# NetManAIOps/ChatTS

Measured on NVIDIA H100. Metric: decode_tokens_per_s, higher is better.
Workload: dtype bf16

## Files before the change

chatts_b200/csrc/common.cuh:

```cuda
#pragma once
#include <cuda.h>
#include <cudaTypedefs.h>
#include <cuda_bf16.h>
#include <cuda_fp16.h>
#include <cuda_runtime.h>
#include <stdint.h>
#include <stdio.h>
#include <string.h>

#include "../../include/chatts_b200.h"

struct cts_ctx {
  int device;
  int sm_count;
  int max_smem_optin;
  char err[512];
  void* scratch;
  size_t scratch_bytes;
  PFN_cuTensorMapEncodeTiled_v12000 encode_tiled;
  int l2_prefetch_mb;
  int no_persistent_gemm;
  int norm_cluster;
  int decode_stages;
  int no_ts_fused;
  int no_next_prefetch;
  int next_prefetch_mb;
};

int cts_set_error(cts_ctx* ctx, int code, const char* fmt, ...);

#define CTS_CHECK_ARG(ctx, cond, msg)                                         \
  do {                                                                        \
    if (!(cond)) return cts_set_error((ctx), CTS_ERR_BAD_ARG, "%s: %s", __func__, (msg)); \
  } while (0)

#define CTS_CUDA(ctx, expr)                                                   \
  do {                                                                        \
    cudaError_t _e = (expr);                                                  \
    if (_e != cudaSuccess)                                                    \
      return cts_set_error((ctx), CTS_ERR_CUDA, "%s: %s -> %s", __func__, #expr, cudaGetErrorString(_e)); \
  } while (0)

#define CTS_LAUNCH_CHECK(ctx)                                                 \
  do {                                                                        \
    cudaError_t _e = cudaGetLastError();                                      \
    if (_e != cudaSuccess)                                                    \
      return cts_set_error((ctx), CTS_ERR_CUDA, "%s: launch -> %s", __func__, cudaGetErrorString(_e)); \
  } while (0)

static inline long long cdiv_ll(long long a, long long b) { return (a + b - 1) / b; }

__device__ __forceinline__ void pdl_wait() { asm volatile("griddepcontrol.wait;" ::: "memory"); }
__device__ __forceinline__ void pdl_trigger() { asm volatile("griddepcontrol.launch_dependents;" ::: "memory"); }

template <typename... KArgs, typename... Args>
static inline cudaError_t launch_pdl(void (*kern)(KArgs...), dim3 grid, dim3 block, size_t smem, cudaStream_t st,
                                     unsigned cluster_x, Args... args) {
  cudaLaunchConfig_t cfg = {};
  cfg.gridDim = grid;
  cfg.blockDim = block;
  cfg.dynamicSmemBytes = smem;
  cfg.stream = st;
  cudaLaunchAttribute attr[2];
  int n = 0;
  attr[n].id = cudaLaunchAttributeProgrammaticStreamSerialization;
  attr[n].val.programmaticStreamSerializationAllowed = 1;
  ++n;
  if (cluster_x > 1) {
    attr[n].id = cudaLaunchAttributeClusterDimension;
    attr[n].val.clusterDim.x = cluster_x;
    attr[n].val.clusterDim.y = 1;
    attr[n].val.clusterDim.z = 1;
    ++n;
  }
  cfg.attrs = attr;
  cfg.numAttrs = n;
  return cudaLaunchKernelEx(&cfg, kern, static_cast<KArgs>(args)...);
}

template <typename T> struct DT;
template <> struct DT<__nv_bfloat16> {
  static __device__ __forceinline__ float to_f(__nv_bfloat16 v) { return __bfloat162float(v); }
  static __device__ __forceinline__ __nv_bfloat16 from_f(float v) { return __float2bfloat16_rn(v); }
};
template <> struct DT<__half> {
  static __device__ __forceinline__ float to_f(__half v) { return __half2float(v); }
  static __device__ __forceinline__ __half from_f(float v) { return __float2half_rn(v); }
};
template <typename T> __device__ __forceinline__ float rnd(float v) { return DT<T>::to_f(DT<T>::from_f(v)); }

template <typename T> __device__ __forceinline__ void unpack8(const uint4& u, float* f) {
  const T* p = reinterpret_cast<const T*>(&u);
#pragma unroll
  for (int i = 0; i < 8; ++i) f[i] = DT<T>::to_f(p[i]);
}
template <typename T> __device__ __forceinline__ uint4 pack8(const float* f) {
  uint4 u;
  T* p = reinterpret_cast<T*>(&u);
#pragma unroll
  for (int i = 0; i < 8; ++i) p[i] = DT<T>::from_f(f[i]);
  return u;
}

__device__ __forceinline__ float warp_sum(float v) {
#pragma unroll
  for (int o = 16; o > 0; o >>= 1) v += __shfl_xor_sync(0xffffffffu, v, o);
  return v;
}
__device__ __forceinline__ float warp_max(float v) {
#pragma unroll
  for (int o = 16; o > 0; o >>= 1) v = fmaxf(v, __shfl_xor_sync(0xffffffffu, v, o));
  return v;
}

__device__ __forceinline__ float gelu_erf(float x) { return 0.5f * x * (1.0f + erff(x * 0.70710678118654752440f)); }
__device__ __forceinline__ float silu_f(float x) { return x / (1.0f + expf(-x)); }

__device__ __forceinline__ uint32_t smem_u32(const void* p) { return (uint32_t)__cvta_generic_to_shared(p); }

__device__ __forceinline__ void mbar_init(uint64_t* bar, uint32_t count) {
  asm volatile("mbarrier.init.shared::cta.b64 [%0], %1;" ::"r"(smem_u32(bar)), "r"(count) : "memory");
}
__device__ __forceinline__ void fence_mbar_init() { asm volatile("fence.mbarrier_init.release.cluster;" ::: "memory"); }
__device__ __forceinline__ void fence_proxy_async_smem() { asm volatile("fence.proxy.async.shared::cta;" ::: "memory"); }

__device__ __forceinline__ void mbar_expect_tx(uint64_t* bar, uint32_t bytes) {
  asm volatile("mbarrier.arrive.expect_tx.shared::cta.b64 _, [%0], %1;" ::"r"(smem_u32(bar)), "r"(bytes) : "memory");
}
__device__ __forceinline__ void mbar_arrive(uint64_t* bar) {
  asm volatile("mbarrier.arrive.shared::cta.b64 _, [%0];" ::"r"(smem_u32(bar)) : "memory");
}
__device__ __forceinline__ bool mbar_try_wait(uint64_t* bar, uint32_t parity) {
  uint32_t ok;
  asm volatile(
      "{\n\t.reg .pred p;\n\t"
      "mbarrier.try_wait.parity.shared::cta.b64 p, [%1], %2;\n\t"
      "selp.u32 %0, 1, 0, p;\n\t}"
      : "=r"(ok)
      : "r"(smem_u32(bar)), "r"(parity)
      : "memory");
  return ok != 0;
}
#ifndef CTS_WAIT_LIMIT
#define CTS_WAIT_LIMIT (1u << 26)
#endif
__device__ __forceinline__ void mbar_wait(uint64_t* bar, uint32_t parity) {
  uint32_t n = 0;
  while (!mbar_try_wait(bar, parity)) {
    if (++n > CTS_WAIT_LIMIT) {
      printf("chatts_b200: mbarrier wait timed out (block %d,%d,%d thread %d)\n", blockIdx.x, blockIdx.y, blockIdx.z,
             threadIdx.x);
      __trap();
    }
  }
}

#define CTS_L2_EVICT_NORMAL 0x1000000000000000ull
#define CTS_L2_EVICT_FIRST 0x12F0000000000000ull
#define CTS_L2_EVICT_LAST 0x14F0000000000000ull

__device__ __forceinline__ void tma_load_2d(void* smem_dst, const CUtensorMap* tm, uint64_t* bar, int c0, int c1,
                                            uint64_t policy) {
  asm volatile(
      "cp.async.bulk.tensor.2d.shared::cluster.global.mbarrier::complete_tx::bytes.L2::cache_hint"
      " [%0], [%1, {%3, %4}], [%2], %5;"
      ::"r"(smem_u32(smem_dst)), "l"(tm), "r"(smem_u32(bar)), "r"(c0), "r"(c1), "l"(policy)
      : "memory");
}
__device__ __forceinline__ void tma_prefetch_l2_2d(const CUtensorMap* tm, int c0, int c1) {
  asm volatile("cp.async.bulk.prefetch.tensor.2d.L2.global.tile [%0, {%1, %2}];" ::"l"(tm), "r"(c0), "r"(c1) : "memory");
}
__device__ __forceinline__ void tma_store_2d(const CUtensorMap* tm, const void* smem_src, int c0, int c1) {
  asm volatile("cp.async.bulk.tensor.2d.global.shared::cta.bulk_group [%0, {%2, %3}], [%1];"
               ::"l"(tm), "r"(smem_u32(smem_src)), "r"(c0), "r"(c1) : "memory");
}
__device__ __forceinline__ void tma_store_commit() { asm volatile("cp.async.bulk.commit_group;" ::: "memory"); }
__device__ __forceinline__ void tma_store_wait_read0() { asm volatile("cp.async.bulk.wait_group 0;" ::: "memory"); }
__device__ __forceinline__ void tma_load_2d_nohint(void* smem_dst, const CUtensorMap* tm, uint64_t* bar, int c0, int c1) {
  asm volatile(
// ... 168 lines not shown
```

chatts_b200/csrc/ctx.cu:

```cuda
#include <stdarg.h>
#include <stdlib.h>

#include "common.cuh"
#include "tensormap.cuh"

int cts_set_error(cts_ctx* ctx, int code, const char* fmt, ...) {
  if (ctx) {
    va_list ap;
    va_start(ap, fmt);
    vsnprintf(ctx->err, sizeof(ctx->err), fmt, ap);
    va_end(ap);
  }
  return code;
}

extern "C" int cts_version(void) { return 100; }

extern "C" const char* cts_arch(void) {
#if defined(CTS_BUILD_ARCH)
  return CTS_BUILD_ARCH;
#else
  return "unknown";
#endif
}

extern "C" int cts_ctx_create(int device, cts_ctx** out) {
  if (!out) return CTS_ERR_BAD_ARG;
  *out = nullptr;
  cts_ctx* ctx = (cts_ctx*)calloc(1, sizeof(cts_ctx));
  if (!ctx) return CTS_ERR_CUDA;
  ctx->device = device;
  cudaError_t e = cudaSetDevice(device);
  if (e != cudaSuccess) {
    fprintf(stderr, "chatts_b200: cudaSetDevice(%d) failed: %s\n", device, cudaGetErrorString(e));
    free(ctx);
    return CTS_ERR_CUDA;
  }
  cudaDeviceProp prop;
  e = cudaGetDeviceProperties(&prop, device);
  if (e != cudaSuccess) {
    free(ctx);
    return CTS_ERR_CUDA;
  }
  if (prop.major != 9 || prop.minor != 0) {
    fprintf(stderr, "chatts_b200: device %d is sm_%d%d; this library contains sm_90a code only\n", device, prop.major,
            prop.minor);
    free(ctx);
    return CTS_ERR_UNSUPPORTED;
  }
  ctx->sm_count = prop.multiProcessorCount;
  ctx->max_smem_optin = (int)prop.sharedMemPerBlockOptin;
  void* fn = nullptr;
  cudaDriverEntryPointQueryResult qres;
  e = cudaGetDriverEntryPoint("cuTensorMapEncodeTiled", &fn, cudaEnableDefault, &qres);
  if (e != cudaSuccess || qres != cudaDriverEntryPointSuccess || !fn) {
    fprintf(stderr, "chatts_b200: cannot resolve cuTensorMapEncodeTiled\n");
    free(ctx);
    return CTS_ERR_CUDA;
  }
  ctx->encode_tiled = (PFN_cuTensorMapEncodeTiled_v12000)fn;
  const char* e1 = getenv("CTS_L2_PREFETCH_MB");
  ctx->l2_prefetch_mb = e1 ? atoi(e1) : 0;
  const char* e4 = getenv("CTS_NO_PERSISTENT_GEMM");
  ctx->no_persistent_gemm = e4 ? atoi(e4) : 0;
  const char* e5 = getenv("CTS_NORM_CLUSTER");
  ctx->norm_cluster = e5 ? atoi(e5) : 8;
  const char* e2 = getenv("CTS_DECODE_SMEM_KB");
  ctx->decode_stages = e2 ? atoi(e2) : 75;
  {
    int cur = 0;
    cudaGetDevice(&cur);
    cudaSetDevice(device);
    ctx->scratch = nullptr;
    ctx->scratch_bytes = 4096;
    if (cudaMalloc(&ctx->scratch, ctx->scratch_bytes) != cudaSuccess || cudaMemset(ctx->scratch, 0, ctx->scratch_bytes) != cudaSuccess) {
      fprintf(stderr, "chatts_b200: cannot allocate the context scratch\n");
      ctx->scratch = nullptr;
    }
    cudaSetDevice(cur);
  }
  const char* e8 = getenv("CTS_TS_FUSED");
  ctx->no_ts_fused = (e8 && atoi(e8) == 0) ? 1 : 0;
  const char* e6 = getenv("CTS_NEXT_PREFETCH");
  ctx->no_next_prefetch = (e6 && atoi(e6) == 0) ? 1 : 0;
  const char* e7 = getenv("CTS_NEXT_PREFETCH_MB");
  ctx->next_prefetch_mb = e7 ? atoi(e7) : 0;
  *out = ctx;
  return CTS_OK;
}

extern "C" void cts_ctx_destroy(cts_ctx* ctx) {
  if (!ctx) return;
  if (ctx->scratch) cudaFree(ctx->scratch);
  free(ctx);
}

extern "C" const char* cts_last_error(const cts_ctx* ctx) { return ctx ? ctx->err : "null ctx"; }

int cts_make_tmap_2d(cts_ctx* ctx, CUtensorMap* tm, const void* base, long long rows, long long cols, long long ld_elems,
                     int box_rows, int is_bf16) {
  if (((uintptr_t)base & 15) != 0) return cts_set_error(ctx, CTS_ERR_BAD_ARG, "tensor map: base not 16-byte aligned");
  if ((ld_elems * 2) % 16 != 0) return cts_set_error(ctx, CTS_ERR_BAD_ARG, "tensor map: row pitch %lld B not a multiple of 16", ld_elems * 2);
  if (box_rows < 1 || box_rows > 256) return cts_set_error(ctx, CTS_ERR_BAD_ARG, "tensor map: box rows %d", box_rows);
  cuuint64_t dims[2] = {(cuuint64_t)cols, (cuuint64_t)rows};
  cuuint64_t strides[1] = {(cuuint64_t)(ld_elems * 2)};
  cuuint32_t box[2] = {64u, (cuuint32_t)box_rows};
  cuuint32_t estr[2] = {1u, 1u};
  CUresult r = ctx->encode_tiled(tm, is_bf16 ? CU_TENSOR_MAP_DATA_TYPE_BFLOAT16 : CU_TENSOR_MAP_DATA_TYPE_FLOAT16, 2,
                                 const_cast<void*>(base), dims, strides, box, estr, CU_TENSOR_MAP_INTERLEAVE_NONE,
                                 CU_TENSOR_MAP_SWIZZLE_128B, CU_TENSOR_MAP_L2_PROMOTION_L2_256B,
                                 CU_TENSOR_MAP_FLOAT_OOB_FILL_NONE);
  if (r != CUDA_SUCCESS) return cts_set_error(ctx, CTS_ERR_CUDA, "cuTensorMapEncodeTiled failed: CUresult %d", (int)r);
  return CTS_OK;
}

int cts_make_tmap_2d_dense(cts_ctx* ctx, CUtensorMap* tm, const void* base, long long rows, long long cols, long long ld_elems,
                           int box_rows, int box_cols, int is_bf16) {
  if (((uintptr_t)base & 15) != 0) return cts_set_error(ctx, CTS_ERR_BAD_ARG, "tensor map: base not 16-byte aligned");
  if ((ld_elems * 2) % 16 != 0) return cts_set_error(ctx, CTS_ERR_BAD_ARG, "tensor map: row pitch %lld B not a multiple of 16", ld_elems * 2);
  if (box_rows < 1 || box_rows > 256 || box_cols < 8 || box_cols > 256 || (box_cols * 2) % 16 != 0)
    return cts_set_error(ctx, CTS_ERR_BAD_ARG, "tensor map: box %d x %d", box_rows, box_cols);
  cuuint64_t dims[2] = {(cuuint64_t)cols, (cuuint64_t)rows};
  cuuint64_t strides[1] = {(cuuint64_t)(ld_elems * 2)};
  cuuint32_t box[2] = {(cuuint32_t)box_cols, (cuuint32_t)box_rows};
  cuuint32_t estr[2] = {1u, 1u};
  CUresult r = ctx->encode_tiled(tm, is_bf16 ? CU_TENSOR_MAP_DATA_TYPE_BFLOAT16 : CU_TENSOR_MAP_DATA_TYPE_FLOAT16, 2,
                                 const_cast<void*>(base), dims, strides, box, estr, CU_TENSOR_MAP_INTERLEAVE_NONE,
                                 CU_TENSOR_MAP_SWIZZLE_NONE, CU_TENSOR_MAP_L2_PROMOTION_L2_256B, CU_TENSOR_MAP_FLOAT_OOB_FILL_NONE);
  if (r != CUDA_SUCCESS) return cts_set_error(ctx, CTS_ERR_CUDA, "cuTensorMapEncodeTiled (dense) failed: CUresult %d", (int)r);
  return CTS_OK;
}

extern "C" int cts_trace_set_gemm(unsigned long long* buf);
extern "C" int cts_trace_set_elementwise(unsigned long long* buf);
extern "C" int cts_trace_set_attention(unsigned long long* buf);
extern "C" int cts_trace_set_allreduce_ll(unsigned long long* buf);
extern "C" int cts_trace_set_fused(unsigned long long* buf);
extern "C" int cts_trace_set_ts_fused(unsigned long long* buf);
extern "C" int cts_trace_set_w4(unsigned long long* buf);
extern "C" int cts_trace_enable(cts_ctx* ctx, unsigned long long* buf) {
  if (!ctx) return CTS_ERR_BAD_ARG;
  if (cts_trace_set_gemm(buf) || cts_trace_set_elementwise(buf) || cts_trace_set_attention(buf) || cts_trace_set_allreduce_ll(buf) || cts_trace_set_fused(buf) || cts_trace_set_ts_fused(buf) || cts_trace_set_w4(buf))
    return cts_set_error(ctx, CTS_ERR_CUDA, "cts_trace_enable: cudaMemcpyToSymbol failed");
  return CTS_OK;
}
```

chatts_b200/csrc/gemm_tcgen05.cu:

```cuda
#include <type_traits>

#include "common.cuh"
#include "tensormap.cuh"
#include "trace.cuh"

namespace {

constexpr int kBM = 128;
constexpr int kBK = 64;
constexpr int kMaxStages = 12;
constexpr int kThreads = 192;

struct GemmParams {
  long long n, k, t, out_ld;
  const void* bias;
  const void* residual;
  void* out;
  const int* row_map;
  int kb_total;
  int split_k;
  int stages;
  int epilogue;
  float* splitk_ws;
  int* tile_cnt;
  int l2_prefetch;
  int staged;
  int next_tiles, next_split, next_kb_total, next_pf;
};

template <int BN, bool DUAL> __host__ __device__ constexpr int stage_bytes() { return kBM * kBK * 2 * (DUAL ? 2 : 1) + BN * kBK * 2; }
template <int BN> __host__ __device__ constexpr bool acc_in_ring() { return BN <= 32; }

template <typename T, int BN, bool DUAL>
__global__ void __launch_bounds__(kThreads, 1)
gemm_tn_kernel(const __grid_constant__ CUtensorMap tm_w, const __grid_constant__ CUtensorMap tm_w2,
               const __grid_constant__ CUtensorMap tm_x, const __grid_constant__ CUtensorMap tm_next, const __grid_constant__ CUtensorMap tm_out,
               const __grid_constant__ CUtensorMap tm_res, const GemmParams p) {
  extern __shared__ uint8_t smem_raw[];
  __shared__ uint64_t full_bar[kMaxStages];
  __shared__ uint64_t empty_bar[kMaxStages];
  __shared__ uint64_t res_bar;
  __shared__ int last_flag;

  constexpr int kStage = stage_bytes<BN, DUAL>();
  constexpr int kABytes = kBM * kBK * 2;
  constexpr int kLd = acc_ld<BN>();
  constexpr bool kIsBf16 = std::is_same<T, __nv_bfloat16>::value;

  const uint32_t raw = smem_u32(smem_raw);
  uint8_t* smem = smem_raw + (((raw + 1023u) & ~1023u) - raw);

  const int warp = threadIdx.x >> 5;
  const int lane = threadIdx.x & 31;
  const int f0 = blockIdx.x * kBM;
  const int t0 = blockIdx.y * BN;
  const int split = blockIdx.z;
  const int stages = p.stages;

  const int kb0 = (int)(((long long)p.kb_total * split) / p.split_k);
  const int kb1 = (int)(((long long)p.kb_total * (split + 1)) / p.split_k);
  const int nkb = kb1 - kb0;

  pdl_trigger();
  if (threadIdx.x == 0) {
    tma_prefetch_desc(&tm_w);
    tma_prefetch_desc(&tm_x);
    if (DUAL) tma_prefetch_desc(&tm_w2);
    for (int s = 0; s < stages; ++s) {
      mbar_init(&full_bar[s], 1);
      mbar_init(&empty_bar[s], 1);
    }
    mbar_init(&res_bar, 1);
    fence_mbar_init();
  }
  __syncthreads();

  if (warp == 4) {
    if (lane == 0) {
      const int npre = nkb < stages ? nkb : stages;
      CTS_TRACE(CTS_TK_GEMM, 0);
      for (int i = 0; i < npre; ++i) {
        mbar_expect_tx(&full_bar[i], (uint32_t)kStage);
        uint8_t* st = smem + (size_t)i * kStage;
        const int kc = (kb0 + i) * kBK;
        tma_load_2d(st, &tm_w, &full_bar[i], kc, f0, CTS_L2_EVICT_FIRST);
        if (DUAL) tma_load_2d(st + kABytes, &tm_w2, &full_bar[i], kc, f0, CTS_L2_EVICT_FIRST);
      }
      {
        const int npf = (nkb - npre) < p.l2_prefetch ? (nkb - npre) : p.l2_prefetch;
        for (int i = npre; i < npre + npf; ++i) {
          tma_prefetch_l2_2d(&tm_w, (kb0 + i) * kBK, f0);
          if (DUAL) tma_prefetch_l2_2d(&tm_w2, (kb0 + i) * kBK, f0);
        }
      }
      pdl_wait();
      CTS_TRACE(CTS_TK_GEMM, 1);
      for (int i = 0; i < npre; ++i) {
        uint8_t* st = smem + (size_t)i * kStage;
        tma_load_2d(st + kABytes * (DUAL ? 2 : 1), &tm_x, &full_bar[i], (kb0 + i) * kBK, t0, CTS_L2_EVICT_LAST);
      }
      for (int i = npre; i < nkb; ++i) {
        const int s = i % stages;
        const uint32_t ph = (uint32_t)(i / stages) & 1u;
        mbar_wait(&empty_bar[s], ph ^ 1u);
        mbar_expect_tx(&full_bar[s], (uint32_t)kStage);
        uint8_t* st = smem + (size_t)s * kStage;
        const int kc = (kb0 + i) * kBK;
        tma_load_2d(st, &tm_w, &full_bar[s], kc, f0, CTS_L2_EVICT_FIRST);
        if (DUAL) tma_load_2d(st + kABytes, &tm_w2, &full_bar[s], kc, f0, CTS_L2_EVICT_FIRST);
        tma_load_2d(st + kABytes * (DUAL ? 2 : 1), &tm_x, &full_bar[s], kc, t0, CTS_L2_EVICT_LAST);
      }
      CTS_TRACE(CTS_TK_GEMM, 2);
      if (p.next_pf > 0) {
        const int units = p.next_tiles * p.next_split;
        const int n_ours = (int)(gridDim.x * gridDim.y * gridDim.z);
        const int c = (int)(blockIdx.x + gridDim.x * (blockIdx.y + gridDim.y * blockIdx.z));
        for (int u = c; u < units; u += n_ours) {
          const int x2 = u % p.next_tiles, z2 = u / p.next_tiles;
          const int kbn0 = (int)(((long long)p.next_kb_total * z2) / p.next_split);
          const int kbn1 = (int)(((long long)p.next_kb_total * (z2 + 1)) / p.next_split);
          const int cnt = (kbn1 - kbn0) < p.next_pf ? (kbn1 - kbn0) : p.next_pf;
          for (int i = 0; i < cnt; ++i) tma_prefetch_l2_2d(&tm_next, (kbn0 + i) * kBK, x2 * kBM);
        }
      }
    }
  } else if (warp < 4) {
    Acc128<BN> acc, acc2;
    acc.zero();
    if (DUAL) acc2.zero();
    for (int i = 0; i < nkb; ++i) {
      const int s = i % stages;
      mbar_wait(&full_bar[s], (uint32_t)(i / stages) & 1u);
      const uint32_t a_addr = smem_u32(smem + (size_t)s * kStage);
      const uint32_t b_addr = a_addr + kABytes * (DUAL ? 2 : 1);
      acc.template mma_kblock<kIsBf16>(a_addr, b_addr, i == 0);
      if (DUAL) acc2.template mma_kblock<kIsBf16>(a_addr + kABytes, b_addr, i == 0);
      wgmma_wait<DUAL ? 2 : 1>();
      if (i > 0 && threadIdx.x == 0) mbar_arrive(&empty_bar[(i - 1) % stages]);
    }
    wgmma_wait<0>();
    if (nkb > 0 && threadIdx.x == 0) mbar_arrive(&empty_bar[(nkb - 1) % stages]);
    named_bar_sync(1, 128);
    float* acc_s = reinterpret_cast<float*>(acc_in_ring<BN>() ? smem : smem + (size_t)stages * kStage);
    acc.store(acc_s, kLd);
    if (DUAL) acc2.store(acc_s + kBM * kLd, kLd);
    pdl_wait();
    named_bar_sync(1, 128);
    const int q = warp & 3;
    const long long f = (long long)f0 + q * 32 + lane;
    const bool f_ok = f < p.n;
    const int row = q * 32 + lane;
    float bias = 0.f;
    if (p.bias != nullptr && f_ok) bias = DT<T>::to_f(reinterpret_cast<const T*>(p.bias)[f]);
    const int epi = p.epilogue;
    if (p.staged) {
      T* out_s = reinterpret_cast<T*>(smem);
      T* res_s = reinterpret_cast<T*>(smem + (size_t)BN * kBM * 2);
      const int ft = q * 32 + lane;
      if (epi == CTS_EPI_RESIDUAL) {
        if (threadIdx.x == 64) {
          mbar_expect_tx(&res_bar, (uint32_t)(BN * kBM * 2));
          tma_load_2d_nohint(res_s, &tm_res, &res_bar, f0, t0);
        }
        mbar_wait(&res_bar, 0);
      }
#pragma unroll 1
      for (int c = 0; c < BN; c += 16) {
        if ((long long)t0 + c >= p.t) break;
        uint32_t v[16], v2[16];
        acc_ld16(acc_s, kLd, row, c, v);
        if (DUAL) acc_ld16(acc_s + kBM * kLd, kLd, row, c, v2);
#pragma unroll
        for (int j = 0; j < 16; ++j) {
          const float acc = __uint_as_float(v[j]);
          float r;
          if (epi == CTS_EPI_SWIGLU) {
            r = rnd<T>(silu_f(rnd<T>(acc))) * rnd<T>(__uint_as_float(v2[j]));
          } else {
            r = acc + bias;
            if (epi == CTS_EPI_GELU) r = gelu_erf(rnd<T>(r));
            else if (epi == CTS_EPI_RESIDUAL) r = rnd<T>(r) + DT<T>::to_f(res_s[(c + j) * kBM + ft]);
          }
          out_s[(c + j) * kBM + ft] = DT<T>::from_f(r);
        }
      }
      fence_proxy_async_smem();
      named_bar_sync(1, 128);
      if (threadIdx.x == 64) {
        tma_store_2d(&tm_out, out_s, f0, t0);
        tma_store_commit();
        tma_store_wait_read0();
      }
    } else if (epi == CTS_EPI_SPLITK_F32) {
      float* dst = p.split_k > 1 ? p.splitk_ws + (long long)split * p.t * p.n : reinterpret_cast<float*>(p.out);
#pragma unroll 1
      for (int c = 0; c < BN; c += 16) {
        if ((long long)t0 + c >= p.t) break;
        uint32_t v[16];
        acc_ld16(acc_s, kLd, row, c, v);
#pragma unroll
        for (int j = 0; j < 16; ++j) {
          const long long t = (long long)t0 + c + j;
          if (t < p.t && f_ok) dst[t * p.n + f] = __uint_as_float(v[j]);
        }
      }
      if (p.split_k > 1) {
        __threadfence();
        named_bar_sync(1, 128);
        const int tile_id = blockIdx.y * gridDim.x + blockIdx.x;
        if (threadIdx.x == 64) last_flag = (atomicAdd(&p.tile_cnt[tile_id], 1) == p.split_k - 1);
        named_bar_sync(1, 128);
        if (last_flag) {
          __threadfence();
          const long long tmax = p.t - t0 < BN ? p.t - t0 : BN;
          if (f_ok) {
            float* o = reinterpret_cast<float*>(p.out);
#pragma unroll 2
            for (long long tt = 0; tt < tmax; ++tt) {
              const long long off = (t0 + tt) * p.n + f;
              float a = 0.f;
              for (int s2 = 0; s2 < p.split_k; ++s2) a += __ldcg(p.splitk_ws + (long long)s2 * p.t * p.n + off);
              o[off] = a;
            }
          }
          if (threadIdx.x == 64) p.tile_cnt[tile_id] = 0;
        }
      }
    } else {
#pragma unroll 1
    for (int c = 0; c < BN; c += 16) {
      if ((long long)t0 + c >= p.t) break;
      uint32_t v[16], v2[16];
      acc_ld16(acc_s, kLd, row, c, v);
      if (DUAL) acc_ld16(acc_s + kBM * kLd, kLd, row, c, v2);
#pragma unroll
      for (int j = 0; j < 16; ++j) {
        const long long t = (long long)t0 + c + j;
        if (t >= p.t || !f_ok) continue;
        const float acc = __uint_as_float(v[j]);
        if (epi == CTS_EPI_PARTIAL_F32) {
          reinterpret_cast<float*>(p.out)[((long long)split * p.t + t) * p.n + f] = acc;
          continue;
        }
        long long row = t;
        if (p.row_map != nullptr) {
          row = p.row_map[t];
          if (row < 0) continue;
        }
        float r;
        if (epi == CTS_EPI_SWIGLU) {
          const float g = rnd<T>(acc);
          const float u = rnd<T>(__uint_as_float(v2[j]));
          r = rnd<T>(silu_f(g)) * u;
        } else {
          r = acc + bias;
          if (epi == CTS_EPI_GELU) {
            r = gelu_erf(rnd<T>(r));
          } else if (epi == CTS_EPI_RESIDUAL) {
            r = rnd<T>(r) + DT<T>::to_f(reinterpret_cast<const T*>(p.residual)[row * p.out_ld + f]);
          }
        }
        reinterpret_cast<T*>(p.out)[row * p.out_ld + f] = DT<T>::from_f(r);
      }
    }
    }
  }

  if (threadIdx.x == 0) CTS_TRACE(CTS_TK_GEMM, 3);
}

constexpr int kPBN = 128;
constexpr int kPStages = 4;
constexpr int kPStageBytes = kBM * kBK * 2 + kPBN * kBK * 2;
constexpr int kPOutBytes = kPBN * kBM * 2;

template <typename T>
__global__ void __launch_bounds__(kThreads, 1)
gemm_tn_persistent_kernel(const __grid_constant__ CUtensorMap tm_w, const __grid_constant__ CUtensorMap tm_x,
                          const __grid_constant__ CUtensorMap tm_out, const __grid_constant__ CUtensorMap tm_res,
                          const GemmParams p) {
  extern __shared__ uint8_t smem_raw[];
  __shared__ uint64_t full_bar[kPStages], empty_bar[kPStages], res_bar;
  constexpr bool kIsBf16 = std::is_same<T, __nv_bfloat16>::value;
  const uint32_t raw = smem_u32(smem_raw);
  uint8_t* smem = smem_raw + (((raw + 1023u) & ~1023u) - raw);
  uint8_t* out_s = smem + kPStages * kPStageBytes;
  uint8_t* res_s = out_s + kPOutBytes;

  const int warp = threadIdx.x >> 5, lane = threadIdx.x & 31;
  const int tiles_m = (int)((p.n + kBM - 1) / kBM), tiles_n = (int)((p.t + kPBN - 1) / kPBN);
  const int total_tiles = tiles_m * tiles_n;
  const int nkb = p.kb_total;
  const int epi = p.epilogue;
  const int gm = p.l2_prefetch > 0 ? p.l2_prefetch : tiles_m;
  auto tile_coords = [&](int id, int& m_blk, int& n_blk) {
    const int per_group = gm * tiles_n;
    const int g = id / per_group, r = id - g * per_group;
    const int gm_here = min(gm, tiles_m - g * gm);
    n_blk = r / gm_here;
    m_blk = g * gm + (r - n_blk * gm_here);
  };

  pdl_trigger();
  if (threadIdx.x == 0) {
    tma_prefetch_desc(&tm_w); tma_prefetch_desc(&tm_x); tma_prefetch_desc(&tm_out);
    for (int s = 0; s < kPStages; ++s) { mbar_init(&full_bar[s], 1); mbar_init(&empty_bar[s], 1); }
    mbar_init(&res_bar, 1);
    fence_mbar_init();
  }
  __syncthreads();

  if (warp == 4) {
    if (lane == 0) {
      pdl_wait();
      uint32_t it = 0;
      for (int tile = blockIdx.x; tile < total_tiles; tile += gridDim.x) {
        int mb, nb;
        tile_coords(tile, mb, nb);
        const int f0 = mb * kBM, t0 = nb * kPBN;
        for (int kb = 0; kb < nkb; ++kb, ++it) {
          const int s = it % kPStages;
          mbar_wait(&empty_bar[s], ((it / kPStages) & 1u) ^ 1u);
          mbar_expect_tx(&full_bar[s], (uint32_t)kPStageBytes);
          uint8_t* st = smem + (size_t)s * kPStageBytes;
          tma_load_2d(st, &tm_w, &full_bar[s], kb * kBK, f0, CTS_L2_EVICT_NORMAL);
          tma_load_2d(st + kBM * kBK * 2, &tm_x, &full_bar[s], kb * kBK, t0, CTS_L2_EVICT_NORMAL);
        }
      }
    }
  } else if (warp < 4) {
    pdl_wait();
    uint32_t it = 0, res_uses = 0;
    T* outp = reinterpret_cast<T*>(out_s);
    const T* resp = reinterpret_cast<const T*>(res_s);
    const T* biasp = reinterpret_cast<const T*>(p.bias);
    for (int tile = blockIdx.x; tile < total_tiles; tile += gridDim.x) {
      int mb, nb;
      tile_coords(tile, mb, nb);
      const int f0 = mb * kBM, t0 = nb * kPBN;
      if (epi == CTS_EPI_RESIDUAL && threadIdx.x == 0) {
        fence_proxy_async_smem();
        mbar_expect_tx(&res_bar, (uint32_t)kPOutBytes);
        tma_load_2d_nohint(res_s, &tm_res, &res_bar, f0, t0);
      }
      Acc128<kPBN> acc;
      acc.zero();
      for (int kb = 0; kb < nkb; ++kb, ++it) {
        const int s = it % kPStages;
        mbar_wait(&full_bar[s], (it / kPStages) & 1u);
        const uint32_t a_addr = smem_u32(smem + (size_t)s * kPStageBytes);
        acc.template mma_kblock<kIsBf16>(a_addr, a_addr + kBM * kBK * 2, kb == 0);
        wgmma_wait<1>();
        if (kb > 0 && threadIdx.x == 0) mbar_arrive(&empty_bar[(it - 1) % kPStages]);
      }
      wgmma_wait<0>();
      if (nkb > 0 && threadIdx.x == 0) mbar_arrive(&empty_bar[(it - 1) % kPStages]);
      if (epi == CTS_EPI_RESIDUAL) {
        mbar_wait(&res_bar, res_uses & 1u);
        ++res_uses;
      }
      if (epi == CTS_EPI_SWIGLU_IL) {
#pragma unroll
        for (int i = 0; i < kPBN / 2; ++i) {
          const float g = rnd<T>(acc.d[0][i]);
          const float u = rnd<T>(acc.d[1][i]);
          outp[acc_col(i) * 64 + acc_row(i)] = DT<T>::from_f(rnd<T>(silu_f(g)) * u);
        }
      } else {
#pragma unroll
        for (int h = 0; h < 2; ++h) {
          float bias[2] = {0.f, 0.f};
#pragma unroll
          for (int e = 0; e < 2; ++e) {
            const long long f = (long long)f0 + 64 * h + acc_row(2 * e);
            if (biasp != nullptr && f < p.n) bias[e] = DT<T>::to_f(biasp[f]);
          }
#pragma unroll
          for (int i = 0; i < kPBN / 2; ++i) {
            const int ft = 64 * h + acc_row(i), tt = acc_col(i);
            float r = acc.d[h][i] + bias[(i >> 1) & 1];
            if (epi == CTS_EPI_GELU) r = gelu_erf(rnd<T>(r));
            else if (epi == CTS_EPI_RESIDUAL) r = rnd<T>(r) + DT<T>::to_f(resp[tt * kBM + ft]);
            outp[tt * kBM + ft] = DT<T>::from_f(r);
          }
        }
      }
      fence_proxy_async_smem();
      named_bar_sync(1, 128);
      if (threadIdx.x == 0) {
        if (epi == CTS_EPI_SWIGLU_IL) tma_store_2d(&tm_out, out_s, f0 / 2, t0);
        else tma_store_2d(&tm_out, out_s, f0, t0);
        tma_store_commit();
        asm volatile("cp.async.bulk.wait_group.read 0;" ::: "memory");
      }
      named_bar_sync(1, 128);
    }
    if (threadIdx.x == 0) tma_store_wait_read0();
  }
}

template <typename T>
int launch_persistent(cts_ctx* ctx, const cts_gemm_args* a, cudaStream_t stream) {
  const bool is_bf16 = a->dtype == CTS_BF16;
  const bool il = a->epilogue == CTS_EPI_SWIGLU_IL;
  CUtensorMap tm_w, tm_x, tm_out, tm_res;
  int rc = cts_make_tmap_2d(ctx, &tm_w, a->w, a->n, a->k, a->w_ld, kBM, is_bf16);
  if (rc) return rc;
  rc = cts_make_tmap_2d(ctx, &tm_x, a->x, a->t, a->k, a->x_ld, kPBN, is_bf16);
  if (rc) return rc;
  rc = cts_make_tmap_2d_dense(ctx, &tm_out, a->out, a->t, il ? a->n / 2 : a->n, a->out_ld, kPBN, il ? 64 : kBM, is_bf16);
  if (rc) return rc;
  tm_res = tm_out;
  if (a->epilogue == CTS_EPI_RESIDUAL) {
    rc = cts_make_tmap_2d_dense(ctx, &tm_res, a->residual, a->t, a->n, a->out_ld, kPBN, kBM, is_bf16);
    if (rc) return rc;
  }
  GemmParams p;
  memset(&p, 0, sizeof(p));
  p.n = a->n; p.k = a->k; p.t = a->t; p.out_ld = a->out_ld;
  p.bias = a->bias; p.residual = a->residual; p.out = a->out;
  p.kb_total = (int)cdiv_ll(a->k, kBK);
  p.split_k = 1; p.epilogue = a->epilogue; p.stages = kPStages;
  {
    const long long tiles_m = cdiv_ll(a->n, kBM);
    long long gmax = (20LL << 20) / ((long long)kBM * a->k * 2);
    if (gmax < 1) gmax = 1;
    const long long groups = cdiv_ll(tiles_m, gmax);
    p.l2_prefetch = (int)cdiv_ll(tiles_m, groups);
    if (ctx->l2_prefetch_mb < 0) p.l2_prefetch = 0;
  }
  const size_t smem = (size_t)kPStages * kPStageBytes + 2 * kPOutBytes + 1024;
  auto kern = gemm_tn_persistent_kernel<T>;
  CTS_CUDA(ctx, cudaFuncSetAttribute(kern, cudaFuncAttributeMaxDynamicSharedMemorySize, (int)smem));
  const long long tiles = cdiv_ll(a->n, kBM) * cdiv_ll(a->t, kPBN);
  const unsigned grid = (unsigned)(tiles < ctx->sm_count ? tiles : ctx->sm_count);
  CTS_CUDA(ctx, launch_pdl(kern, dim3(grid), dim3(kThreads), smem, stream, 1, tm_w, tm_x, tm_out, tm_res, p));
  return CTS_OK;
}

template <typename T, int BN, bool DUAL>
int launch(cts_ctx* ctx, const cts_gemm_args* a, cudaStream_t stream) {
  const bool is_bf16 = a->dtype == CTS_BF16;
  CUtensorMap tm_w, tm_w2, tm_x;
  int rc = cts_make_tmap_2d(ctx, &tm_w, a->w, a->n, a->k, a->w_ld, kBM, is_bf16);
  if (rc) return rc;
  if (DUAL) {
    rc = cts_make_tmap_2d(ctx, &tm_w2, a->w2, a->n, a->k, a->w_ld, kBM, is_bf16);
    if (rc) return rc;
  } else {
    tm_w2 = tm_w;
  }
  rc = cts_make_tmap_2d(ctx, &tm_x, a->x, a->t, a->k, a->x_ld, BN, is_bf16);
  if (rc) return rc;
  const bool staged = BN >= 64 && a->row_map == nullptr && a->epilogue != CTS_EPI_PARTIAL_F32 && a->epilogue != CTS_EPI_SPLITK_F32 && (a->out_ld * 2) % 16 == 0 &&
                      ((uintptr_t)a->out & 15) == 0 && (a->epilogue != CTS_EPI_RESIDUAL || ((uintptr_t)a->residual & 15) == 0);
  CUtensorMap tm_out = tm_x, tm_res = tm_x;
  if (staged) {
    rc = cts_make_tmap_2d_dense(ctx, &tm_out, a->out, a->t, a->n, a->out_ld, BN, kBM, is_bf16);
    if (rc) return rc;
    if (a->epilogue == CTS_EPI_RESIDUAL) {
      rc = cts_make_tmap_2d_dense(ctx, &tm_res, a->residual, a->t, a->n, a->out_ld, BN, kBM, is_bf16);
      if (rc) return rc;
    }
  }

  GemmParams p;
  p.n = a->n; p.k = a->k; p.t = a->t; p.out_ld = a->out_ld;
  p.bias = a->bias; p.residual = a->residual; p.out = a->out; p.row_map = a->row_map;
  p.splitk_ws = (float*)a->splitk_ws; p.tile_cnt = a->tile_counters;
  p.kb_total = (int)cdiv_ll(a->k, kBK);
  p.split_k = a->split_k;
  p.epilogue = a->epilogue;
  CUtensorMap tm_next = tm_w;
  p.next_tiles = p.next_split = p.next_kb_total = p.next_pf = 0;
  if (BN <= 32 && a->next_w != nullptr && a->next_prefetch_bytes > 0 && a->next_n > 0 && a->next_k > 0 && a->next_split >= 1 && !ctx->no_next_prefetch) {
    rc = cts_make_tmap_2d(ctx, &tm_next, a->next_w, a->next_n, a->next_k, a->next_ld > 0 ? a->next_ld : a->next_k, kBM, is_bf16);
    if (rc) return rc;
    p.next_tiles = (int)cdiv_ll(a->next_n, kBM);
    p.next_split = a->next_split;
    p.next_kb_total = (int)cdiv_ll(a->next_k, kBK);
    const long long units = (long long)p.next_tiles * p.next_split;
    long long pf = a->next_prefetch_bytes / (units * kBM * kBK * 2);
    const long long per_unit = cdiv_ll(p.next_kb_total, p.next_split);
    if (pf > per_unit) pf = per_unit;
    p.next_pf = (int)pf;
  }
  constexpr int kStage = stage_bytes<BN, DUAL>();
  const int budget = (BN <= 32) ? ctx->decode_stages * 1024 : (BN <= 128 ? 100 * 1024 : 200 * 1024);
  int stages = budget / kStage;
  if (stages > kMaxStages) stages = kMaxStages;
  if (stages < 2) stages = 2;
  p.stages = stages;
  p.staged = staged ? 1 : 0;
  p.l2_prefetch = 0;
  if (BN <= 32 && ctx->l2_prefetch_mb > 0) {
    const long long ctas = cdiv_ll(a->n, kBM) * cdiv_ll(a->t, BN) * a->split_k;
    const long long per = ((long long)ctx->l2_prefetch_mb << 20) / (ctas * kBM * kBK * 2 * (DUAL ? 2 : 1));
    p.l2_prefetch = (int)(per > 64 ? 64 : per);
  }
  if (staged && stages * kStage < 2 * BN * kBM * 2) stages = (2 * BN * kBM * 2 + kStage - 1) / kStage;
  p.stages = stages;
  const size_t acc_bytes = (size_t)acc_smem_bytes<BN>() * (DUAL ? 2 : 1);
  const size_t ring = (size_t)stages * kStage;
  const size_t smem = (acc_in_ring<BN>() ? (ring > acc_bytes ? ring : acc_bytes) : ring + acc_bytes) + 1024;
  auto kern = gemm_tn_kernel<T, BN, DUAL>;
  CTS_CUDA(ctx, cudaFuncSetAttribute(kern, cudaFuncAttributeMaxDynamicSharedMemorySize, (int)smem));
  dim3 grid((unsigned)cdiv_ll(a->n, kBM), (unsigned)cdiv_ll(a->t, BN), (unsigned)a->split_k);
  CTS_CUDA(ctx, launch_pdl(kern, grid, dim3(kThreads), smem, stream, 1, tm_w, tm_w2, tm_x, tm_next, tm_out, tm_res, p));
  return CTS_OK;
}

template <typename T, bool DUAL>
int dispatch_bn(cts_ctx* ctx, const cts_gemm_args* a, cudaStream_t stream) {
  const long long t = a->t;
  if (t <= 16) return launch<T, 16, DUAL>(ctx, a, stream);
  if (t <= 32) return launch<T, 32, DUAL>(ctx, a, stream);
  if (t <= 64 || DUAL) return launch<T, 64, DUAL>(ctx, a, stream);
  return launch<T, 128, false>(ctx, a, stream);
}

}

extern "C" int cts_gemm(cts_ctx* ctx, const cts_gemm_args* a, void* stream) {
  if (!ctx) return CTS_ERR_BAD_ARG;
  CTS_CHECK_ARG(ctx, a != nullptr, "null args");
  CTS_CHECK_ARG(ctx, a->w && a->x && a->out, "null w/x/out");
  CTS_CHECK_ARG(ctx, a->n > 0 && a->k > 0 && a->t > 0, "n, k, t must be positive");
  CTS_CHECK_ARG(ctx, a->dtype == CTS_BF16 || a->dtype == CTS_F16, "dtype must be CTS_BF16 or CTS_F16");
  CTS_CHECK_ARG(ctx, a->epilogue >= CTS_EPI_NONE && a->epilogue <= CTS_EPI_SWIGLU_IL, "unknown epilogue");
  CTS_CHECK_ARG(ctx, a->split_k >= 1, "split_k must be >= 1");
  CTS_CHECK_ARG(ctx, a->split_k == 1 || a->epilogue == CTS_EPI_PARTIAL_F32 || a->epilogue == CTS_EPI_SPLITK_F32,
                "split_k > 1 needs CTS_EPI_PARTIAL_F32 or CTS_EPI_SPLITK_F32");
  CTS_CHECK_ARG(ctx, a->epilogue != CTS_EPI_SPLITK_F32 || a->split_k == 1 || (a->splitk_ws && a->tile_counters),
                "CTS_EPI_SPLITK_F32 with split_k > 1 needs splitk_ws and tile_counters");
  CTS_CHECK_ARG(ctx, a->split_k <= cdiv_ll(a->k, kBK), "split_k exceeds the number of 64-wide K blocks");
  CTS_CHECK_ARG(ctx, a->split_k <= 65535 && cdiv_ll(a->t, 16) <= 65535 * 16LL, "grid too large");
  CTS_CHECK_ARG(ctx, (a->epilogue == CTS_EPI_SWIGLU) == (a->w2 != nullptr), "w2 is required by (and only by) CTS_EPI_SWIGLU");
  CTS_CHECK_ARG(ctx, a->epilogue != CTS_EPI_RESIDUAL || a->residual != nullptr, "CTS_EPI_RESIDUAL needs residual");
  CTS_CHECK_ARG(ctx, a->w_ld >= a->k && a->x_ld >= a->k, "leading dimension smaller than k");
  CTS_CHECK_ARG(ctx, a->epilogue == CTS_EPI_PARTIAL_F32 || a->epilogue == CTS_EPI_SPLITK_F32 ||
                         a->out_ld >= (a->epilogue == CTS_EPI_SWIGLU_IL ? a->n / 2 : a->n), "out_ld smaller than n");
  cudaStream_t st = (cudaStream_t)stream;
  CTS_CHECK_ARG(ctx, a->epilogue != CTS_EPI_SWIGLU_IL || (a->n % 128 == 0 && a->t > 128 && a->row_map == nullptr),
                "CTS_EPI_SWIGLU_IL needs n % 128 == 0, t > 128 and no row_map (small t: CTS_EPI_PARTIAL_F32 + cts_reduce_swiglu)");
  const bool pers_epi = a->epilogue == CTS_EPI_NONE || a->epilogue == CTS_EPI_GELU || a->epilogue == CTS_EPI_RESIDUAL ||
                        a->epilogue == CTS_EPI_SWIGLU_IL;
  if (a->t > 128 && pers_epi && a->row_map == nullptr && a->split_k == 1 && (a->out_ld * 2) % 16 == 0 &&
      ((uintptr_t)a->out & 15) == 0 && (a->epilogue != CTS_EPI_RESIDUAL || ((uintptr_t)a->residual & 15) == 0) &&
      !ctx->no_persistent_gemm) {
    return a->dtype == CTS_BF16 ? launch_persistent<__nv_bfloat16>(ctx, a, st) : launch_persistent<__half>(ctx, a, st);
  }
  CTS_CHECK_ARG(ctx, a->epilogue != CTS_EPI_SWIGLU_IL, "CTS_EPI_SWIGLU_IL is only implemented by the persistent kernel");
  const bool dual = a->epilogue == CTS_EPI_SWIGLU;
  if (a->dtype == CTS_BF16)
    return dual ? dispatch_bn<__nv_bfloat16, true>(ctx, a, st) : dispatch_bn<__nv_bfloat16, false>(ctx, a, st);
  return dual ? dispatch_bn<__half, true>(ctx, a, st) : dispatch_bn<__half, false>(ctx, a, st);
}

extern "C" int cts_gemm_suggest_split(cts_ctx* ctx, long long n, long long k, long long t, int dual) {
  if (!ctx || n <= 0 || k <= 0 || t <= 0) return 1;
  const int bn = t <= 16 ? 16 : t <= 32 ? 32 : t <= 64 ? 64 : 128;
  const long long tiles = cdiv_ll(dual ? 2 * n : n, kBM) * cdiv_ll(t, bn);
  const long long kb = cdiv_ll(k, kBK);
  const long long slots = (long long)ctx->sm_count * (bn <= 128 ? (dual && bn <= 32 ? 3 : 2) : 1);
  if (tiles >= slots) return 1;
  long long s = slots / tiles;
  const long long per_split_min = bn <= 32 ? 2 : 8;
  const long long max_by_k = kb / per_split_min > 0 ? kb / per_split_min : 1;
  if (s > max_by_k) s = max_by_k;
  if (s > 16) s = 16;
  if (s < 1) s = 1;
  return (int)s;
}

CTS_TRACE_SETTER(cts_trace_set_gemm)
```

Baseline: 2524.

## Add persistent weight-streaming GEMM kernel for small-token decode shapes

Adds a persistent decode GEMM for t <= 32 with no-epilogue or partial-f32 output. It runs a grid of a few CTAs per SM that walk (tile, split) work units through a deep TMA ring, so weight loads for the next units are issued ahead of compute and can cross tile boundaries. A dedicated producer warp issues weight loads before the PDL wait, and the consumer warpgroup runs wgmma on 64- or 128-row tiles. The old per-CTA L2 prefetch of weight blocks is removed. The kernel waits on wgmma after each stage, and its epilogue uses scalar global stores, which may limit gains on small shapes.

Result: faster. 2617, median of 6 (+3.7%).

```diff
diff --git a/chatts_b200/csrc/common.cuh b/chatts_b200/csrc/common.cuh
--- a/chatts_b200/csrc/common.cuh
+++ b/chatts_b200/csrc/common.cuh
@@ -25,6 +25,10 @@
   int no_ts_fused;
   int no_next_prefetch;
   int next_prefetch_mb;
+  int no_stream_gemm;
+  int stream_ctas;
+  int stream_rows;
+  int stream_kblocks;
 };
 
 int cts_set_error(cts_ctx* ctx, int code, const char* fmt, ...);
diff --git a/chatts_b200/csrc/ctx.cu b/chatts_b200/csrc/ctx.cu
--- a/chatts_b200/csrc/ctx.cu
+++ b/chatts_b200/csrc/ctx.cu
@@ -85,6 +85,14 @@
   ctx->no_next_prefetch = (e6 && atoi(e6) == 0) ? 1 : 0;
   const char* e7 = getenv("CTS_NEXT_PREFETCH_MB");
   ctx->next_prefetch_mb = e7 ? atoi(e7) : 0;
+  const char* e9 = getenv("CTS_NO_STREAM_GEMM");
+  ctx->no_stream_gemm = e9 ? atoi(e9) : 0;
+  const char* e10 = getenv("CTS_STREAM_CTAS");
+  ctx->stream_ctas = e10 ? atoi(e10) : 2;
+  const char* e11 = getenv("CTS_STREAM_ROWS");
+  ctx->stream_rows = e11 ? atoi(e11) : 128;
+  const char* e12 = getenv("CTS_STREAM_KBLOCKS");
+  ctx->stream_kblocks = e12 ? atoi(e12) : 1;
   *out = ctx;
   return CTS_OK;
 }
diff --git a/chatts_b200/csrc/gemm_tcgen05.cu b/chatts_b200/csrc/gemm_tcgen05.cu
--- a/chatts_b200/csrc/gemm_tcgen05.cu
+++ b/chatts_b200/csrc/gemm_tcgen05.cu
@@ -85,13 +85,6 @@
         const int kc = (kb0 + i) * kBK;
         tma_load_2d(st, &tm_w, &full_bar[i], kc, f0, CTS_L2_EVICT_FIRST);
         if (DUAL) tma_load_2d(st + kABytes, &tm_w2, &full_bar[i], kc, f0, CTS_L2_EVICT_FIRST);
-      }
-      {
-        const int npf = (nkb - npre) < p.l2_prefetch ? (nkb - npre) : p.l2_prefetch;
-        for (int i = npre; i < npre + npf; ++i) {
-          tma_prefetch_l2_2d(&tm_w, (kb0 + i) * kBK, f0);
-          if (DUAL) tma_prefetch_l2_2d(&tm_w2, (kb0 + i) * kBK, f0);
-        }
       }
       pdl_wait();
       CTS_TRACE(CTS_TK_GEMM, 1);
@@ -269,6 +262,154 @@
   if (threadIdx.x == 0) CTS_TRACE(CTS_TK_GEMM, 3);
 }
 
+constexpr int kSMaxStages = 16;
+constexpr int kSThreads = 160;
+
+struct StreamParams {
+  long long n, t, out_ld;
+  const void* bias;
+  void* out;
+  int kb_total, split_k, tiles, stages, epilogue;
+};
+
+template <int BN, int H, int KS> __host__ __device__ constexpr int stream_stage_bytes() { return KS * (H * 64 + BN) * kBK * 2; }
+
+template <typename T, int BN, int H, int KS>
+__global__ void __launch_bounds__(kSThreads, 1)
+gemm_stream_kernel(const __grid_constant__ CUtensorMap tm_w, const __grid_constant__ CUtensorMap tm_x, const StreamParams p) {
+  extern __shared__ uint8_t smem_raw[];
+  __shared__ uint64_t full_bar[kSMaxStages];
+  __shared__ uint64_t empty_bar[kSMaxStages];
+
+  constexpr int kRows = 64 * H;
+  constexpr int kWBlk = kRows * kBK * 2;
+  constexpr int kXBlk = BN * kBK * 2;
+  constexpr int kStage = stream_stage_bytes<BN, H, KS>();
+  constexpr bool kIsBf16 = std::is_same<T, __nv_bfloat16>::value;
+
+  const uint32_t raw = smem_u32(smem_raw);
+  uint8_t* ring = smem_raw + (((raw + 1023u) & ~1023u) - raw);
+  const int warp = threadIdx.x >> 5, lane = threadIdx.x & 31;
+  const int S = p.stages;
+  const int units = p.tiles * p.split_k;
+  auto unit = [&](int u, int& tile, int& split, int& kb0, int& kb1) {
+    tile = u % p.tiles;
+    split = u / p.tiles;
+    kb0 = (int)(((long long)p.kb_total * split) / p.split_k);
+    kb1 = (int)(((long long)p.kb_total * (split + 1)) / p.split_k);
+  };
+
+  pdl_trigger();
+  if (threadIdx.x == 0) {
+    tma_prefetch_desc(&tm_w);
+    tma_prefetch_desc(&tm_x);
+    for (int s = 0; s < S; ++s) {
+      mbar_init(&full_bar[s], 1);
+      mbar_init(&empty_bar[s], 1);
+    }
+    fence_mbar_init();
+  }
+  __syncthreads();
+
+  if (warp == 4) {
+    if (lane == 0) {
+      auto issue_w = [&](int s, int f0, int kb, int nb) {
+        mbar_expect_tx(&full_bar[s], (uint32_t)(nb * (kWBlk + kXBlk)));
+        uint8_t* st = ring + (size_t)s * kStage;
+        for (int b = 0; b < nb; ++b) tma_load_2d(st + b * kWBlk, &tm_w, &full_bar[s], (kb + b) * kBK, f0, CTS_L2_EVICT_FIRST);
+      };
+      int pre = 0;
+      for (int u = blockIdx.x; u < units && pre < S; u += gridDim.x) {
+        int tile, split, kb0, kb1;
+        unit(u, tile, split, kb0, kb1);
+        for (int kb = kb0; kb < kb1 && pre < S; kb += KS, ++pre) issue_w(pre, tile * kRows, kb, min(KS, kb1 - kb));
+      }
+      pdl_wait();
+      int s = 0, n = 0;
+      uint32_t ph = 1u;
+      for (int u = blockIdx.x; u < units; u += gridDim.x) {
+        int tile, split, kb0, kb1;
+        unit(u, tile, split, kb0, kb1);
+        for (int kb = kb0; kb < kb1; kb += KS, ++n) {
+          const int nb = min(KS, kb1 - kb);
+          if (n >= pre) {
+            mbar_wait(&empty_bar[s], ph);
+            issue_w(s, tile * kRows, kb, nb);
+          }
+          uint8_t* xs = ring + (size_t)s * kStage + KS * kWBlk;
+          for (int b = 0; b < nb; ++b) tma_load_2d(xs + b * kXBlk, &tm_x, &full_bar[s], (kb + b) * kBK, 0, CTS_L2_EVICT_LAST);
+          if (++s == S) { s = 0; ph ^= 1u; }
+        }
+      }
+    }
+  } else {
+    pdl_wait();
+    Acc128<BN> acc;
+    float (&d)[2][BN / 2] = acc.d;
+    int s = 0;
+    uint32_t ph = 0u;
+    for (int u = blockIdx.x; u < units; u += gridDim.x) {
+      int tile, split, kb0, kb1;
+      unit(u, tile, split, kb0, kb1);
+      for (int kb = kb0; kb < kb1; kb += KS) {
+        const int nb = min(KS, kb1 - kb);
+        mbar_wait(&full_bar[s], ph);
+        const uint32_t wa = smem_u32(ring + (size_t)s * kStage), xa = wa + KS * kWBlk;
+        if constexpr (H == 2) {
+#pragma unroll
+          for (int b = 0; b < KS; ++b)
+            if (b < nb) acc.template mma_kblock<kIsBf16>(wa + b * kWBlk, xa + b * kXBlk, kb == kb0 && b == 0);
+        } else {
+          for (int i = 0; i < BN / 2; ++i) wgmma_fence_operand(d[0][i]);
+          wgmma_fence();
+#pragma unroll
+          for (int b = 0; b < KS; ++b) {
+            if (b < nb) {
+              const uint64_t ad = gmma_desc_k_sw128(wa + b * kWBlk), bd = gmma_desc_k_sw128(xa + b * kXBlk);
+#pragma unroll
+              for (int kk = 0; kk < 4; ++kk)
+                wgmma_m64k16<BN, kIsBf16>(d[0], ad + 2 * kk, bd + 2 * kk, (kb == kb0 && b == 0 && kk == 0) ? 0 : 1);
+            }
+          }
+          wgmma_commit();
+          for (int i = 0; i < BN / 2; ++i) wgmma_fence_operand(d[0][i]);
+        }
+        wgmma_wait<0>();
+        if (threadIdx.x == 0) mbar_arrive(&empty_bar[s]);
+        if (++s == S) { s = 0; ph ^= 1u; }
+      }
+      const long long f0 = (long long)tile * kRows;
+      if (p.epilogue == CTS_EPI_PARTIAL_F32) {
+        float* dst = reinterpret_cast<float*>(p.out) + (long long)split * p.t * p.n;
+#pragma unroll
+        for (int h = 0; h < H; ++h)
+#pragma unroll
+          for (int i = 0; i < BN / 2; ++i) {
+            const long long f = f0 + 64 * h + acc_row(i), t = acc_col(i);
+            if (t < p.t && f < p.n) dst[t * p.n + f] = d[h][i];
+          }
+      } else {
+        T* dst = reinterpret_cast<T*>(p.out);
+        const T* bias = reinterpret_cast<const T*>(p.bias);
+#pragma unroll
+        for (int h = 0; h < H; ++h)
+#pragma unroll
+          for (int e = 0; e < 2; ++e) {
+            const long long f = f0 + 64 * h + acc_row(2 * e);
+            const float bv = (bias != nullptr && f < p.n) ? DT<T>::to_f(bias[f]) : 0.f;
+#pragma unroll
+            for (int i = 2 * e; i < BN / 2; i += 4)
+#pragma unroll
+              for (int j = 0; j < 2; ++j) {
+                const long long t = acc_col(i + j);
+                if (t < p.t && f < p.n) dst[t * p.out_ld + f] = DT<T>::from_f(d[h][i + j] + bv);
+              }
+          }
+      }
+    }
+  }
+}
+
 constexpr int kPBN = 128;
 constexpr int kPStages = 4;
 constexpr int kPStageBytes = kBM * kBK * 2 + kPBN * kBK * 2;
@@ -493,11 +634,6 @@
   p.stages = stages;
   p.staged = staged ? 1 : 0;
   p.l2_prefetch = 0;
-  if (BN <= 32 && ctx->l2_prefetch_mb > 0) {
-    const long long ctas = cdiv_ll(a->n, kBM) * cdiv_ll(a->t, BN) * a->split_k;
-    const long long per = ((long long)ctx->l2_prefetch_mb << 20) / (ctas * kBM * kBK * 2 * (DUAL ? 2 : 1));
-    p.l2_prefetch = (int)(per > 64 ? 64 : per);
-  }
   if (staged && stages * kStage < 2 * BN * kBM * 2) stages = (2 * BN * kBM * 2 + kStage - 1) / kStage;
   p.stages = stages;
   const size_t acc_bytes = (size_t)acc_smem_bytes<BN>() * (DUAL ? 2 : 1);
@@ -508,6 +644,65 @@
   dim3 grid((unsigned)cdiv_ll(a->n, kBM), (unsigned)cdiv_ll(a->t, BN), (unsigned)a->split_k);
   CTS_CUDA(ctx, launch_pdl(kern, grid, dim3(kThreads), smem, stream, 1, tm_w, tm_w2, tm_x, tm_next, tm_out, tm_res, p));
   return CTS_OK;
+}
+
+struct StreamCfg { int off, ctas, rows, kblocks; };
+static inline StreamCfg stream_cfg(const cts_ctx* ctx) {
+#ifndef CTS_HOST_SHIM
+  return {ctx->no_stream_gemm, ctx->stream_ctas, ctx->stream_rows, ctx->stream_kblocks};
+#else
+  auto env = [](const char* name, int dflt) { const char* e = getenv(name); return e ? atoi(e) : dflt; };
+  return {env("CTS_NO_STREAM_GEMM", 0), env("CTS_STREAM_CTAS", 2), env("CTS_STREAM_ROWS", 128), env("CTS_STREAM_KBLOCKS", 1)};
+#endif
+}
+
+template <typename T, int BN, int H, int KS>
+int launch_stream(cts_ctx* ctx, const StreamCfg& cfg, const cts_gemm_args* a, cudaStream_t stream) {
+  const bool is_bf16 = a->dtype == CTS_BF16;
+  CUtensorMap tm_w, tm_x;
+  int rc = cts_make_tmap_2d(ctx, &tm_w, a->w, a->n, a->k, a->w_ld, 64 * H, is_bf16);
+  if (rc) return rc;
+  rc = cts_make_tmap_2d(ctx, &tm_x, a->x, a->t, a->k, a->x_ld, BN, is_bf16);
+  if (rc) return rc;
+  StreamParams p;
+  p.n = a->n; p.t = a->t; p.out_ld = a->out_ld;
+  p.bias = a->bias; p.out = a->out;
+  p.kb_total = (int)cdiv_ll(a->k, kBK);
+  p.split_k = a->split_k;
+  p.tiles = (int)cdiv_ll(a->n, 64 * H);
+  p.epilogue = a->epilogue;
+  constexpr int kStage = stream_stage_bytes<BN, H, KS>();
+  const int ctas = cfg.ctas;
+  const int budget = (ctx->max_smem_optin + 1024) / ctas - 3 * 1024;
+  int stages = (budget - 1024) / kStage;
+  if (stages > kSMaxStages) stages = kSMaxStages;
+  if (stages < 2)
+    return cts_set_error(ctx, CTS_ERR_BAD_ARG, "cts_gemm: %d CTAs per SM leave room for fewer than two %d KB stages", ctas, kStage / 1024);
+  p.stages = stages;
+  const size_t smem = (size_t)stages * kStage + 1024;
+  auto kern = gemm_stream_kernel<T, BN, H, KS>;
+  CTS_CUDA(ctx, cudaFuncSetAttribute(kern, cudaFuncAttributeMaxDynamicSharedMemorySize, (int)smem));
+#ifndef CTS_HOST_SHIM
+  CTS_CUDA(ctx, cudaFuncSetAttribute(kern, cudaFuncAttributePreferredSharedMemoryCarveout, (int)cudaSharedmemCarveoutMaxShared));
+#endif
+  const long long units = (long long)p.tiles * p.split_k;
+  long long grid = (long long)ctas * ctx->sm_count;
+  if (grid > units) grid = units;
+  CTS_CUDA(ctx, launch_pdl(kern, dim3((unsigned)grid), dim3(kSThreads), smem, stream, 1, tm_w, tm_x, p));
+  return CTS_OK;
+}
+
+template <typename T, int BN>
+int dispatch_stream(cts_ctx* ctx, const StreamCfg& c, const cts_gemm_args* a, cudaStream_t st) {
+  const int ks = c.kblocks;
+  if (c.rows == 64)
+    return ks == 1 ? launch_stream<T, BN, 1, 1>(ctx, c, a, st) : ks == 2 ? launch_stream<T, BN, 1, 2>(ctx, c, a, st) : launch_stream<T, BN, 1, 4>(ctx, c, a, st);
+  return ks == 1 ? launch_stream<T, BN, 2, 1>(ctx, c, a, st) : ks == 2 ? launch_stream<T, BN, 2, 2>(ctx, c, a, st) : launch_stream<T, BN, 2, 4>(ctx, c, a, st);
+}
+
+template <typename T>
+int dispatch_stream_bn(cts_ctx* ctx, const StreamCfg& c, const cts_gemm_args* a, cudaStream_t st) {
+  return a->t <= 16 ? dispatch_stream<T, 16>(ctx, c, a, st) : dispatch_stream<T, 32>(ctx, c, a, st);
 }
 
 template <typename T, bool DUAL>
@@ -541,6 +736,14 @@
   CTS_CHECK_ARG(ctx, a->epilogue == CTS_EPI_PARTIAL_F32 || a->epilogue == CTS_EPI_SPLITK_F32 ||
                          a->out_ld >= (a->epilogue == CTS_EPI_SWIGLU_IL ? a->n / 2 : a->n), "out_ld smaller than n");
   cudaStream_t st = (cudaStream_t)stream;
+  const bool next_hint = a->next_w != nullptr && a->next_prefetch_bytes > 0;
+  const StreamCfg cfg = stream_cfg(ctx);
+  if (a->t <= 32 && (a->epilogue == CTS_EPI_PARTIAL_F32 || (a->epilogue == CTS_EPI_NONE && a->split_k == 1)) && a->row_map == nullptr &&
+      a->w2 == nullptr && !next_hint && !cfg.off) {
+    CTS_CHECK_ARG(ctx, cfg.ctas >= 1 && cfg.ctas <= 4 && (cfg.rows == 64 || cfg.rows == 128) && (cfg.kblocks == 1 || cfg.kblocks == 2 || cfg.kblocks == 4),
+                  "decode GEMM shape: CTS_STREAM_CTAS 1..4, CTS_STREAM_ROWS 64 or 128, CTS_STREAM_KBLOCKS 1, 2 or 4");
+    return a->dtype == CTS_BF16 ? dispatch_stream_bn<__nv_bfloat16>(ctx, cfg, a, st) : dispatch_stream_bn<__half>(ctx, cfg, a, st);
+  }
   CTS_CHECK_ARG(ctx, a->epilogue != CTS_EPI_SWIGLU_IL || (a->n % 128 == 0 && a->t > 128 && a->row_map == nullptr),
                 "CTS_EPI_SWIGLU_IL needs n % 128 == 0, t > 128 and no row_map (small t: CTS_EPI_PARTIAL_F32 + cts_reduce_swiglu)");
   const bool pers_epi = a->epilogue == CTS_EPI_NONE || a->epilogue == CTS_EPI_GELU || a->epilogue == CTS_EPI_RESIDUAL ||
```
